# gkv856/speaker_embedding_GE2E_loss

Hardware: NVIDIA B200
Metric: GE2E fwd+bwd utterances/s (higher is better)
Workload: dtype tf32

## Files before the change

### speaker_embedding_ge2e_loss_b200/csrc/ge2e_tc.cu

```cuda
#include <cuda.h>
#include <cuda_fp16.h>
#include <cudaTypedefs.h>
#include <limits.h>
#include <stdlib.h>

#include <algorithm>
#include <cstring>
#include <type_traits>
#include <vector>

#include "ge2e_common.cuh"
#include "ge2e_tc_ptx.cuh"

namespace ge2e {

namespace {

using namespace ptx;

constexpr int kTile = 128;
constexpr int kUnit = 128;
constexpr int kSlabCols = 32;
constexpr int kSlabBytes = kTile * 128;
constexpr int kMaxSlabs = 8;
// ... 402 lines not shown
        if (DBG && (dbg & 8)) tr.mark();
        tc_fence_after();
      };
      auto next_bar = [&]() { return bar(BAR_FULL + (stage + 1 == kStages ? 0 : stage + 1)); };
      auto next_par = [&]() { return static_cast<uint32_t>(stage + 1 == kStages ? (phase ^ 1) : phase); };
      auto stage_done = [&](uint32_t probe) {
        __syncwarp();
        ready = __shfl_sync(0xffffffffu, probe, leader) != 0;
        advance();
      };
      auto mma1_stage = [&](uint32_t d_tmem, uint32_t idesc1, int rows_cta, int ks0, int nslab, bool first_of_seg) {
        if (kOpF16) {
          if (first_of_seg) {
            for (int sl = 0; sl < nslab; ++sl) {
              const int s = ks0 + sl, c = s % hs;
              mbar_wait(bar(BAR_A_FULL + c), sg & 1);
              if (kPlanes == 2 && s < hs) mbar_wait(bar(BAR_A_FULL + hs + c), sg & 1);
            }
          }
          stage_wait();
          uint32_t probe = 0;
          if (elect_leader(leader)) {
            probe = mbar_test(next_bar(), next_par());
            for (int sl = 0; sl < nslab; ++sl) {
              const int s = ks0 + sl, c = s % hs;
              const uint64_t db = dk | ((ring_smem + stage * kStageBytes + sl * rows_cta * 128) >> 4);
              umma_f16_ss4<CG>(d_tmem, dk | ((a_smem + c * kSlabBytes) >> 4), db, idesc1, s != 0);
              if (kPlanes == 2 && s < hs)
                umma_f16_ss4<CG>(d_tmem, dk | ((a_smem + (hs + c) * kSlabBytes) >> 4), db, idesc1, 1);
            }
            commit(BAR_EMPTY + stage);
          }
          stage_done(probe);
          return;
        }
        if (first_of_seg) {
          for (int sl = 0; sl < nslab; ++sl) mbar_wait(bar(BAR_A_FULL + ks0 + sl), sg & 1);
        }
        stage_wait();
        uint32_t probe = 0;
        if (elect_leader(leader)) {
          const uint64_t da = dk | ((a_smem + ks0 * kSlabBytes) >> 4);
          const uint64_t db = dk | ((ring_smem + stage * kStageBytes) >> 4);
          const uint32_t eb = bar(BAR_EMPTY + stage);
          if (nslab == 2)
            probe = umma_stage_ss<CG, 2>(d_tmem, da, db, kSlabBytes >> 4, static_cast<uint32_t>(rows_cta * 128) >> 4,
                                         idesc1, ks0 != 0, eb, next_bar(), next_par());
          else
            probe = umma_stage_ss<CG, 1>(d_tmem, da, db, 0, 0, idesc1, ks0 != 0, eb, next_bar(), next_par());
        }
        stage_done(probe);
      };
      const uint32_t idesc_unit = kOpF16 ? idesc_f16(kTile * CG, kUnit, 0, 0) : idesc_tf32(kTile * CG, kUnit, 0, 0);
      auto mma1_unit = [&](int iter, bool first_of_seg) {
        const uint32_t d_tmem = tmem + (iter & 1) * kUnit;
        for (int ks = 0; ks < oslabs; ks += 2)
          mma1_stage(d_tmem, idesc_unit, kUnit / CG, ks, min(2, oslabs - ks), first_of_seg);
        if (elect_one()) commit(BAR_S_FULL + (iter & 1));
        __syncwarp();
      };
      auto mma2_unit = [&](int iter, bool first) {
        const uint32_t a_tmem = tmem + (iter & 1) * kUnit;
        const uint32_t d_tmem = tmem + 2 * kUnit;
        for (int kc = 0; kc < kUnit / kM2; ++kc) {
          stage_wait();
          uint32_t probe = 0;
          if (PREC == PREC_F16) {
            if (elect_leader(leader)) {
              probe = mbar_test(next_bar(), next_par());
              const uint32_t a_hi = a_tmem + 64 * kc;
              const uint64_t db_hi = dmn | ((ring_smem + stage * kStageBytes) >> 4);
              umma_f16_ts2<CG>(d_tmem, a_hi, db_hi, idesc2, !(first && kc == 0));
              umma_f16_ts2<CG>(d_tmem, a_hi + 16, db_hi + 256, idesc2, 1);
              commit(BAR_EMPTY + stage);
            }
            stage_done(probe);
            continue;
          }
          if (kSplit) {
            if (elect_leader(leader)) {
              probe = mbar_test(next_bar(), next_par());
              const uint32_t a_hi = a_tmem + 64 * (kc >> 1) + 16 * (kc & 1), a_lo = a_hi + 32;
              const uint32_t sb = ring_smem + stage * kStageBytes;
              const uint64_t db_hi = dmn | (sb >> 4);
              const uint64_t db_lo = dmn | ((sb + (hs / CG) * kMma2Rows * 128) >> 4);
              umma_f16_ts2<CG>(d_tmem, a_hi, db_hi, idesc2, !(first && kc == 0));
              if (kPlanes == 2) {
                umma_f16_ts2<CG>(d_tmem, a_hi, db_lo, idesc2, 1);
                umma_f16_ts2<CG>(d_tmem, a_lo, db_hi, idesc2, 1);
              }
              commit(BAR_EMPTY + stage);
            }
            stage_done(probe);
            continue;
          }
          if (elect_leader(leader)) {
            const uint64_t db = dmn | ((ring_smem + stage * kStageBytes) >> 4);
            static_assert(kMma2Rows == 32, "umma_stage_ts issues 4 MMAs of 8 k-rows");
            probe = umma_stage_ts<CG>(d_tmem, a_tmem + kc * kMma2Rows, db, idesc2, !(first && kc == 0),
                                      bar(BAR_EMPTY + stage), next_bar(), next_par());
          }
          stage_done(probe);
        }
      };
      Walk wk = make_walk();
      int kind, og, s0, s1;
      for (; wk.next(p, kind, og, s0, s1); ++sg) {
        if (!kBwd) {
          for (int u = s0; u < s1; u += kStepUnits, ++it) {
            const int nu = min(kStepUnits, s1 - u);
            mbar_wait(bar(BAR_S_EMPTY + (it & 1)), ((it >> 1) & 1) ^ 1);
            tc_fence_after();
            const uint32_t d_tmem = tmem + (it & 1) * (kStepUnits * kUnit);
            const uint32_t idesc_step = kOpF16 ? idesc_f16(kTile * CG, nu * kUnit, 0, 0)
                                               : idesc_tf32(kTile * CG, nu * kUnit, 0, 0);
            for (int ks = 0; ks < oslabs; ++ks) mma1_stage(d_tmem, idesc_step, nu * kUnit / CG, ks, 1, u == s0);
            if (elect_one()) commit(BAR_S_FULL + (it & 1));
            __syncwarp();
            tr.mark();
          }
          if (elect_one()) commit(BAR_A_EMPTY);
          __syncwarp();
        } else {
          mma1_unit(it, true);
          for (int i = 0; i < s1 - s0; ++i, ++it) {
            if (i + 1 < s1 - s0) {
              mma1_unit(it + 1, false);
            } else {
              if (elect_one()) commit(BAR_A_EMPTY);
              __syncwarp();
            }
            tr.mark();
            if (i == 0 && sg > 0) { mbar_wait(bar(BAR_ACC_EMPTY), (sg - 1) & 1); tc_fence_after(); }
            mbar_wait(bar(BAR_G_FULL + (it & 1)), (it >> 1) & 1);
            tc_fence_after();
            tr.mark();
            mma2_unit(it, i == 0);
            tr.mark();
          }
          if (elect_one()) commit(BAR_ACC_FULL);
          __syncwarp();
        }
      }
    }
  } else if (warp >= kEpiWarp0) {
    const int ew = warp - kEpiWarp0;
    const int et = tid - kEpiWarp0 * 32;
    const int quarter = ew & 3, half = ew >> 2;
    const int trow = quarter * 32 + lane;
    const uint32_t lane_addr = static_cast<uint32_t>(quarter * 32) << 16;
    const float w = __ldg(p.w), b = __ldg(p.b), eps = p.eps;
    const float w2 = w * kLog2e, b2 = fmaf(w, eps, b) * kLog2e;
    const float bb = fmaf(w, eps, b);
    const float g = (kBwd && !RG && p.grad_out != nullptr) ? __ldg(p.grad_out) : 1.f;
    const float wg = w * g;
    float gamma = 1.f, inv_gamma = 1.f;
    auto gsign_of = [&](int buf, int w) -> uint32_t {
      if constexpr (RG) return tail->gsign[buf][w]; else return 0u;
    };
    const float m2 = b2 + fabsf(w2), c0 = -fabsf(w2);
    float dw_acc = 0.f, db_acc = 0.f, loss_acc = 0.f;
    int it = 0;
    const bool close_here = kBwd && !kSplit && (p.phases & PASS_ROWS);
    Tracer<DBG> tr((trow == 0 && half == 0) ? p.trace : nullptr, 2, kBwd ? 3 : 0);
    tr.mark();
    const uint32_t s_empty0 = lbar(BAR_S_EMPTY), g_full0 = lbar(BAR_G_FULL), acc_empty = lbar(BAR_ACC_EMPTY);
    auto arrive_leader = [&](uint32_t addr) {
      if (CG == 1) mbar_arrive(addr); else mbar_arrive_cluster(addr);
    };
    auto spin_until = [&](const int* ctr, int target) {
      unsigned long long t0 = 0;
      for (unsigned spins = 0;; ++spins) {
        int v;
        asm volatile("ld.acquire.gpu.global.s32 %0, [%1];" : "=r"(v) : "l"(ctr) : "memory");
        if (v >= target) break;
        if ((spins & 1023u) == 1023u) {
          const unsigned long long t = globaltimer_ns();
          if (t0 == 0) t0 = t;
          else if (t - t0 > 2000000000ull) __trap();
        }
      }
    };
    bool zero_seen = false;
    auto wait_zero_fill = [&]() {
      if (zero_seen) return;
      spin_until(p.ctr, static_cast<int>(gridDim.x));
      asm volatile("fence.proxy.async;" ::: "memory");
      zero_seen = true;
    };
    if (kBwd) {
      auto zfill = [&](float4* base, long long n4) {
        const long long z0 = n4 * blockIdx.x / gridDim.x, z1 = n4 * (blockIdx.x + 1) / gridDim.x;
        for (long long i = z0 + et; i < z1; i += kEpiThreads) base[i] = make_float4(0.f, 0.f, 0.f, 0.f);
      };
      if (p.zero_n4 > 0) zfill(p.zero_base, p.zero_n4);
      if (p.zero2_n4 > 0) zfill(p.zero2_base, p.zero2_n4);
      if (close_here) zfill(reinterpret_cast<float4*>(p.rowsum), (p.n_own[SEG_DE] + 3) / 4);
      if (et == 0) tail->rows_all_done = 0;
      __threadfence();
      named_bar_sync(1, kEpiThreads);
      if (et == 0) atomicAdd(p.ctr, 1);
    }

    int lift2 = kSplitLift;
    auto close_row = [&](int r) {
      const float cdv = __ldg(p.cos_diag + r);
      float stat, q;
      if (close_here) {
        const RowClose rc = close_softmax_row_log2(m2, __ldcg(p.rowsum + r), fmaf(cdv, w2, b2),
                                                   fmaf(w, cdv + eps, b), eps);
        stat = rc.stat; q = rc.q;
        p.row_stat_out[r] = stat;
        p.row_aux_out[r] = q;
        p.row_scale_out[r] = w / rc.z;
        if (p.per_row_out != nullptr) p.per_row_out[r] = rc.per;
        loss_acc += rc.per;
      } else {
        stat = __ldg(p.row_stat + r);
        q = __ldg(p.row_aux + r);
        if (kSplit && (p.phases & PASS_ROWS))
          p.row_scale_out[r] = w * exp2f(static_cast<float>(-(kSplitLift + split_extra_lift(q))));
      }
      if (p.phases & PASS_CENTROIDS) {
        if (RG) {
          const float gr = __ldg(p.grad_rows + r);
          dw_acc = fmaf(-q * gr, cdv + eps, dw_acc);
          db_acc -= gr * eps * expf(-stat);
        } else {
          dw_acc = fmaf(-q, cdv + eps, dw_acc);
          db_acc -= eps * expf(-stat);
        }
      }
    };
    auto close_rows = [&]() {
      const int U = p.n_own[SEG_DE];
      if (kSplit && (p.phases & PASS_CENTROIDS)) {
        if (RG) {
          float qm = 0.f, gm = 0.f;
          for (int r = et; r < U; r += kEpiThreads) {
            const float ga = fabsf(__ldg(p.grad_rows + r));
            qm = fmaxf(qm, __ldg(p.row_aux + r) * ga);
            gm = fmaxf(gm, ga);
          }
          qm = warp_max(qm);
          gm = warp_max(gm);
          if (lane == 0) { tail->red[ew] = qm; tail->red[kEpiWarps + ew] = gm; }
          named_bar_sync(1, kEpiThreads);
          qm = tail->red[0];
          gm = tail->red[kEpiWarps];
          for (int i = 1; i < kEpiWarps; ++i) { qm = fmaxf(qm, tail->red[i]); gm = fmaxf(gm, tail->red[kEpiWarps + i]); }
          gamma = gm;
          inv_gamma = gm > 0.f ? 1.f / gm : 0.f;
          lift2 = kSplitLift + split_extra_lift(qm * inv_gamma);
        } else {
          float qm = 0.f;
          for (int r = et; r < U; r += kEpiThreads) qm = fmaxf(qm, __ldg(p.row_aux + r));
          qm = warp_max(qm);
          if (lane == 0) tail->red[ew] = qm;
          named_bar_sync(1, kEpiThreads);
          qm = tail->red[0];
          for (int i = 1; i < kEpiWarps; ++i) qm = fmaxf(qm, tail->red[i]);
          lift2 = kSplitLift + split_extra_lift(qm);
        }
        named_bar_sync(1, kEpiThreads);
      }
      for (int r = blockIdx.x * kEpiThreads + et; r < U; r += gridDim.x * kEpiThreads) close_row(r);
      tr.mark();
    };
    static_assert(kUnit == kTile, "a pass-2 stream unit must be exactly one pass-1 owner tile");
    unsigned long long ready_wait_ns = 0;
    auto tile_ready = [&](int u) {
      if (*reinterpret_cast<volatile int*>(&tail->rows_all_done) != 0) return true;
      int v;
      asm volatile("ld.acquire.gpu.global.s32 %0, [%1];" : "=r"(v) : "l"(p.ctr + 2) : "memory");
      if (v >= p.OT[SEG_DE]) { tail->rows_all_done = 1; return true; }
      asm volatile("ld.acquire.gpu.global.s32 %0, [%1];" : "=r"(v) : "l"(p.seg_done + u) : "memory");
      return v >= p.ST[SEG_DE];
    };
    auto wait_tile = [&](int u) {
      if (tile_ready(u)) return;
      const unsigned long long t0 = DBG ? globaltimer_ns() : 0ull;
      spin_until(p.seg_done + u, p.ST[SEG_DE]);
      if (DBG) ready_wait_ns += globaltimer_ns() - t0;
    };
    bool closed = false;
    int sg_dc0 = -1;

    Walk wk = make_walk();
    int kind, og, s0, s1;
    for (int sg = 0; wk.next(p, kind, og, s0, s1); ++sg) {
      const bool is_dc = kBwd && kind == SEG_DC;
      if (kBwd && !close_here && is_dc && !closed) { close_rows(); closed = true; }
      if (DBG && is_dc && sg_dc0 < 0) { sg_dc0 = sg; tr.put(kTraceEvents - 2, globaltimer_ns()); }
      const int n_str = p.n_str[kind];
      const int ot = og * CG + cr;
      const bool tile_valid = ot < p.OT[kind];
      const int orow = ot * kTile + trow;
      const bool ovalid = orow < p.n_own[kind];
      int jg = -1;
      float cd = 0.f;
      int dlo = 0, dhi = 0;
      if (!is_dc) {
        if (ovalid) {
          jg = p.spk_offset + orow / p.M;
          if (!kBwd) cd = __ldg(p.cos_diag + orow);
        }
      } else {
        const int jl = orow - p.spk_offset;
        if (ovalid && jl >= 0 && (long long)jl * p.M < n_str) { dlo = jl * p.M; dhi = dlo + p.M; }
      }
      const float xd2 = fmaf(cd, w2, b2);
      float m2r = xd2, lsum = 0.f;
      float best = -INFINITY; int bestk = INT_MAX;
      float rs_acc = 0.f;
      float dw_seg = 0.f;
      auto lse2_of = [&](bool valid, float raw, float cdv) -> float {
        if (!valid) return INFINITY;
        if (!close_here) return raw * kLog2e;
        return close_softmax_row_log2(m2, raw, fmaf(cdv, w2, b2), fmaf(w, cdv + eps, b), eps).lse2;
      };
      auto lse2_raw = [&](int ur, float& raw, float& cdv) -> bool {
        if (ur >= n_str) return false;
        if (close_here) { raw = __ldcg(p.rowsum + ur); cdv = __ldg(p.cos_diag + ur); }
        else { raw = __ldg(p.row_stat + ur); cdv = 0.f; }
        return true;
      };
      float c0r = 0.f;
      if (kBwd && kSplit && !is_dc)
        c0r = ovalid ? (b2 + static_cast<float>(kSplitLift + split_extra_lift(__ldg(p.row_aux + orow)))) -
                           __ldg(p.row_stat + orow) * kLog2e
                     : -INFINITY;
      auto grad_of = [&](int ur) -> float { return (RG && ur < n_str) ? __ldg(p.grad_rows + ur) : 0.f; };
      auto stage_row = [&](int buf, bool valid, float raw, float cdv, float gr) {
        float l = lse2_of(valid, raw, cdv);
        if constexpr (RG) {
          l -= log2f(fabsf(gr) * inv_gamma);
          const uint32_t neg = __ballot_sync(0xffffffffu, gr < 0.f);
          if (lane == 0) tail->gsign[buf][quarter] = neg;
        }
        tail->lse_s[buf][trow] = l;
      };
      auto stage_lse = [&](int u, int buf) {
        if (close_here) wait_tile(u);
        float raw = 0.f, cdv = 0.f;
        const bool v = lse2_raw(u * kUnit + trow, raw, cdv);
        stage_row(buf, v, raw, cdv, grad_of(u * kUnit + trow));
      };
      if (is_dc && half == 0) stage_lse(wk.unit(0, s0, s1), it & 1);
      bool deferred = false;

      for (int i = 0; i < s1 - s0; i += kStepUnits, ++it) {
        const int u = wk.unit(i, s0, s1);
        const int nu = min(kStepUnits, s1 - s0 - i);
        const int buf = it & 1;
        float nraw = 0.f, ncd = 0.f, ngr = 0.f;
        bool nvalid = false;
        if (is_dc) {
          if (half == 0 && deferred) { stage_lse(u, buf); deferred = false; }
          named_bar_sync(1, kEpiThreads);
          if (half == 0 && i + 1 < s1 - s0) {
            const int un = wk.unit(i + 1, s0, s1);
            if (!close_here || tile_ready(un)) {
              nvalid = lse2_raw(un * kUnit + trow, nraw, ncd);
// ... 65 lines not shown
        for (int ch = half * nch; ch < (half + 1) * nch; ++ch) {
          const int cc = u * kUnit + ch * 32;
          uint32_t v[32];
          tmem_ld32(t_addr + ch * 32, v);
          tmem_ld_wait();
          if (!kBwd) {
            if (cc < n_str) {
              const bool tailc = cc + 32 > n_str;
              const bool diagc = static_cast<unsigned>(jg - cc) < 32u;
              if (VARIANT == GE2E_SOFTMAX) {
                float x[32];
#pragma unroll
                for (int i = 0; i < 32; ++i) x[i] = fmaf(__uint_as_float(v[i]), w2, b2);
                if (__any_sync(0xffffffffu, tailc || diagc)) {
#pragma unroll
                  for (int i = 0; i < 32; ++i)
                    if (cc + i == jg || cc + i >= n_str) x[i] = -INFINITY;
                }
                float cm = x[0];
#pragma unroll
                for (int i = 1; i < 32; ++i) cm = fmaxf(cm, x[i]);
                const float mn = fmaxf(m2r, cm);
                float sacc = 0.f;
#pragma unroll
                for (int i = 0; i < 32; ++i) sacc += ex2(x[i] - mn);
                lsum = fmaf(lsum, ex2(m2r - mn), sacc);
                m2r = mn;
              } else {
#pragma unroll
                for (int i = 0; i < 32; ++i) {
                  float sv = fmaf(__uint_as_float(v[i]), w, bb);
                  if (cc + i == jg || cc + i >= n_str) sv = -INFINITY;
                  if (sv > best) { best = sv; bestk = cc + i; }
                }
              }
            }
          } else {
            uint32_t gq[32];
            if (!is_dc) {
              const bool special = (cc + 32 > n_str) || (static_cast<unsigned>(jg - cc) < 32u);
              const bool any_special = __any_sync(0xffffffffu, special);
#pragma unroll
              for (int i = 0; i < 32; ++i) {
                float pr = ex2(fmaf(__uint_as_float(v[i]), w2, c0));
                if (any_special && (cc + i >= n_str || cc + i == jg)) pr = 0.f;
                rs_acc += pr;
                gq[i] = __float_as_uint(round_tf32(pr));
              }
            } else {
              const float4* ls4 = reinterpret_cast<const float4*>(&tail->lse_s[buf][ch * 32]);
              const uint32_t neg = gsign_of(buf, ch);
              const bool special = (cc < dhi) && (cc + 32 > dlo);
              const bool any_special = __any_sync(0xffffffffu, special);
#pragma unroll
              for (int i4 = 0; i4 < 8; ++i4) {
                const float4 l4 = ls4[i4];
                const float ls[4] = {l4.x, l4.y, l4.z, l4.w};
#pragma unroll
                for (int q = 0; q < 4; ++q) {
                  const int i = i4 * 4 + q;
                  const float dot = __uint_as_float(v[i]);
                  float pr = ex2(fmaf(dot, w2, b2) - ls[q]);
                  if (any_special && cc + i >= dlo && cc + i < dhi) pr = 0.f;
                  if (RG && ((neg >> i) & 1u)) pr = -pr;
                  dw_seg = fmaf(pr, dot + eps, dw_seg);
                  gq[i] = __float_as_uint(round_tf32(wg * pr));
                }
              }
            }
            tmem_st32(t_addr + ch * 32, gq);
          }
        }
        tr.mark();
        if (!kBwd) {
          tc_fence_before();
          __syncwarp();
          if (lane == 0) arrive_leader(s_empty0 + 8u * buf);
        } else {
          if (is_dc && half == 0 && i + 1 < s1 - s0 && !deferred) stage_row(buf ^ 1, nvalid, nraw, ncd, ngr);
          tmem_st_wait();
          tc_fence_before();
          __syncwarp();
          if (lane == 0) arrive_leader(g_full0 + 8u * buf);
        }
      }

      const bool full = (s0 == 0 && s1 == p.ST[kind]);
      if (!kBwd) {
        float2 mine;
        if (VARIANT == GE2E_SOFTMAX) mine = make_float2(m2r, lsum);
        else mine = make_float2(best, __int_as_float(bestk));
        if (half == 1) tail->xch[trow] = mine;
        named_bar_sync(1, kEpiThreads);
        const float2 theirs = tail->xch[trow];
        named_bar_sync(1, kEpiThreads);
        if (half == 0 && tile_valid) {
          auto fold = [&](float2 q) {
            if (VARIANT == GE2E_SOFTMAX) {
              const float mn = fmaxf(m2r, q.x);
              lsum = lsum * ex2(m2r - mn) + q.y * ex2(q.x - mn);
              m2r = mn;
            } else {
              const int qk = __float_as_int(q.y);
              if (q.x > best || (q.x == best && qk < bestk)) { best = q.x; bestk = qk; }
            }
          };
          fold(theirs);
          const int st = p.ST[SEG_DE];
          const int first_cl = cluster_of_pair(static_cast<long long>(og) * st, p.GP, NC);
          bool last = full;
          if (!full) {
            float2 part;
            if (VARIANT == GE2E_SOFTMAX) part = make_float2(m2r, lsum);
            else part = make_float2(best, __int_as_float(bestk));
            p.seg_part[(static_cast<size_t>(ot) * p.maxseg + (cl - first_cl)) * kTile + trow] = part;
            __threadfence();
            named_bar_sync(2, kTile);
            if (trow == 0) {
              const int done = atomicAdd(p.seg_done + ot, s1 - s0) + (s1 - s0);
              tail->flag = (done == st);
              if (done == st) p.seg_done[ot] = 0;
            }
            named_bar_sync(2, kTile);
            last = tail->flag != 0;
            if (last) {
              __threadfence();
              const int last_cl = cluster_of_pair(static_cast<long long>(og) * st + st - 1, p.GP, NC);
              const int nseg = last_cl - first_cl + 1;
              m2r = xd2; lsum = 0.f; best = -INFINITY; bestk = INT_MAX;
              for (int sgi = 0; sgi < nseg; ++sgi)
                fold(__ldcg(&p.seg_part[(static_cast<size_t>(ot) * p.maxseg + sgi) * kTile + trow]));
            }
          }
          if (last && ovalid) {
            const float Sd = fmaf(w, cd + eps, b);
            float per, stat, aux = 0.f;
            int ks = -1;
            if (VARIANT == GE2E_SOFTMAX) {
              const RowClose rc = close_softmax_row_log2(m2r, lsum, xd2, Sd, eps);
              stat = rc.stat; aux = rc.q; per = rc.per;
            } else {
              per = 1.f - 1.f / (1.f + expf(-Sd));
              stat = best;
              if (bestk != INT_MAX) { ks = bestk; per += 1.f / (1.f + expf(-best)); }
            }
            p.row_stat_out[orow] = stat;
            if (p.row_aux_out != nullptr) p.row_aux_out[orow] = aux;
            if (VARIANT == GE2E_CONTRAST && p.kstar_out != nullptr) p.kstar_out[orow] = ks;
            if (p.per_row_out != nullptr) p.per_row_out[orow] = per;
            loss_acc += per;
          }
        }
      } else {
        if (!is_dc && !close_here) {
        } else if (!is_dc) {
          if (et == 0) wait_zero_fill();
          named_bar_sync(1, kEpiThreads);
          if (ovalid) {
            const float old = atomicAdd(p.rowsum + orow, rs_acc);
            asm volatile("" ::"f"(old));
          }
          named_bar_sync(1, kEpiThreads);
          if (et == 0) {
            bool last = false;
            if (tile_valid) {
              __threadfence();
              last = atomicAdd(p.seg_done + ot, s1 - s0) + (s1 - s0) == p.ST[SEG_DE];
              if (last) { __threadfence(); atomicAdd(p.ctr + 2, 1); }
            }
            tail->flag = last;
          }
          named_bar_sync(1, kEpiThreads);
          if (tail->flag != 0) {
            __threadfence();
            if (et < kTile && ot * kTile + et < p.n_own[SEG_DE]) close_row(ot * kTile + et);
          }
          if (DBG && wk.kind == SEG_DE && wk.gp >= wk.end) tr.put(kTraceEvents - 3, globaltimer_ns());
        } else if (ovalid) {
          if (RG && kSplit) dw_acc += dw_seg * (exp2f(static_cast<float>(-lift2)) * gamma);
          else dw_acc += kSplit ? dw_seg * exp2f(static_cast<float>(-lift2)) : dw_seg;
        }
        mbar_wait(bar(BAR_ACC_FULL), sg & 1);
        tc_fence_after();
        tr.mark();
        fence_proxy_async_smem();
        const int ch0 = half ? kslabs / 2 : 0, ch1 = half ? kslabs : kslabs / 2;
        for (int ch = ch0; ch < ch1; ++ch) {
          uint32_t v[32];
          tmem_ld32(tmem + lane_addr + 2 * kUnit + ch * 32, v);
          tmem_ld_wait();
          if (kSplit && is_dc) {
            const float fs = (RG ? wg * gamma : wg) * exp2f(static_cast<float>(-lift2));
#pragma unroll
            for (int i = 0; i < 32; ++i) v[i] = __float_as_uint(__uint_as_float(v[i]) * fs);
          }
          const uint32_t row_smem = a_smem + ch * kSlabBytes + trow * 128;
#pragma unroll
          for (int c = 0; c < 8; ++c)
            asm volatile("st.shared.v4.b32 [%0], {%1, %2, %3, %4};" ::"r"(row_smem + ((c ^ (trow & 7)) << 4)),
                         "r"(v[4 * c]), "r"(v[4 * c + 1]), "r"(v[4 * c + 2]), "r"(v[4 * c + 3])
                         : "memory");
        }
        tc_fence_before();
        __syncwarp();
        if (lane == 0) arrive_leader(acc_empty);
        tr.mark();
        fence_proxy_async_smem();
        named_bar_sync(1, kEpiThreads);
        if (et == 0) {
          if (tile_valid) {
            const CUtensorMap* tm_out = &tms.out[kind];
            int row0 = ot * kTile;
            bool store = full;
            if (is_dc && p.peer_rows > 0) {
              const int r = row0 / p.peer_rows;
              tm_out = &tms.out_peer[r];
              row0 -= r * p.peer_rows;
              store = false;
            } else if (!full) {
              wait_zero_fill();
            }
            for (int ks = 0; ks < kslabs; ++ks) {
              if (store) tma_store_2d(tm_out, ks * kSlabCols, row0, a_smem + ks * kSlabBytes);
              else tma_reduce_add_2d(tm_out, ks * kSlabCols, row0, a_smem + ks * kSlabBytes);
              tma_store_commit();
            }
          }
          for (int ks = 0; ks < kslabs; ++ks) {
            if (tile_valid) tma_store_wait_read_pending(kslabs - 1 - ks);
            mbar_arrive(bar(BAR_A_FREE + ks));
          }
        }
      }
      tr.mark();
    }
    if (kBwd && !close_here && !closed) close_rows();
    if (DBG && kBwd) tr.put(kTraceEvents - 1, ready_wait_ns);

    if (!kBwd) {
      loss_acc = warp_sum(loss_acc);
      if (lane == 0) tail->red[ew] = loss_acc;
      named_bar_sync(1, kEpiThreads);
      if (ew == 0 && lane == 0) {
        float t = 0.f;
        for (int i = 0; i < kEpiWarps; ++i) t += tail->red[i];
        atomicAdd(p.loss_accum, t);
      }
    } else {
      loss_acc = warp_sum(loss_acc);
      dw_acc = warp_sum(dw_acc) * g;
      db_acc = warp_sum(db_acc) * g;
      if (lane == 0) { tail->red3[ew] = loss_acc; tail->red3[kEpiWarps + ew] = dw_acc; tail->red3[2 * kEpiWarps + ew] = db_acc; }
      named_bar_sync(1, kEpiThreads);
      if (et == 0) {
        float tl = 0.f, tw = 0.f, tb = 0.f;
        for (int i = 0; i < kEpiWarps; ++i) {
          tl += tail->red3[i]; tw += tail->red3[kEpiWarps + i]; tb += tail->red3[2 * kEpiWarps + i];
        }
        if (close_here) atomicAdd(p.loss_accum, tl);
        if (p.phases & PASS_CENTROIDS) { atomicAdd(p.dwdb + 0, tw); atomicAdd(p.dwdb + 1, tb); }
        if (p.stamps != nullptr) p.stamps[2 * blockIdx.x + 1] = globaltimer_ns();
        const bool last_out = atomicAdd(p.ctr + 1, 1) == static_cast<int>(gridDim.x) - 1;
        if (last_out) { atomicExch(p.ctr, 0); atomicExch(p.ctr + 1, 0); atomicExch(p.ctr + 2, 0); }
        tail->flag = last_out;
      }
      named_bar_sync(1, kEpiThreads);
      if (close_here && tail->flag != 0)
        for (int t = et; t < p.OT[SEG_DE]; t += kEpiThreads) p.seg_done[t] = 0;
    }
  }

  tc_fence_before();
  __syncthreads();
  if (CG > 1) cluster_sync_all();
  if (warp == 2) {
    if (CG == 1) tmem_dealloc<512>(tmem); else tmem_dealloc_2cta<512>(tmem);
  }
}

PFN_cuTensorMapEncodeTiled_v12000 get_encode() {
  static PFN_cuTensorMapEncodeTiled_v12000 fn = nullptr;
  if (fn == nullptr) {
    void* ptr = nullptr;
    cudaDriverEntryPointQueryResult qres;
    if (cudaGetDriverEntryPoint("cuTensorMapEncodeTiled", &ptr, cudaEnableDefault, &qres) == cudaSuccess &&
        qres == cudaDriverEntryPointSuccess)
      fn = reinterpret_cast<PFN_cuTensorMapEncodeTiled_v12000>(ptr);
  }
  return fn;
}

struct MapKey {
  const void* base; int rows, D, box, dims;
  bool operator==(const MapKey& o) const {
    return base == o.base && rows == o.rows && D == o.D && box == o.box && dims == o.dims;
  }
};
constexpr int kMapCache = 32;
struct MapCache { MapKey key[kMapCache]; CUtensorMap map[kMapCache]; int next = 0, used = 0; };
thread_local MapCache g_maps;

bool map_lookup(const MapKey& k, CUtensorMap* m) {
  for (int i = 0; i < g_maps.used; ++i)
    if (g_maps.key[i] == k) { *m = g_maps.map[i]; return true; }
  return false;
}
void map_store(const MapKey& k, const CUtensorMap& m) {
  g_maps.key[g_maps.next] = k;
  g_maps.map[g_maps.next] = m;
  g_maps.next = (g_maps.next + 1) % kMapCache;
  g_maps.used = std::min(g_maps.used + 1, kMapCache);
}

int make_map_2d(CUtensorMap* m, const float* base, int rows, int D, int box_rows) {
  const MapKey key{base, rows, D, box_rows, 2};
  if (map_lookup(key, m)) return GE2E_OK;
  auto enc = get_encode();
  if (enc == nullptr) return GE2E_ERR_LAUNCH;
  cuuint64_t dims[2] = {static_cast<cuuint64_t>(D), static_cast<cuuint64_t>(rows)};
  cuuint64_t strides[1] = {static_cast<cuuint64_t>(D) * 4};
  cuuint32_t box[2] = {kSlabCols, static_cast<cuuint32_t>(box_rows)};
  cuuint32_t estr[2] = {1, 1};
  CUresult r = enc(m, CU_TENSOR_MAP_DATA_TYPE_FLOAT32, 2, const_cast<float*>(base), dims, strides, box, estr,
                   CU_TENSOR_MAP_INTERLEAVE_NONE, CU_TENSOR_MAP_SWIZZLE_128B, CU_TENSOR_MAP_L2_PROMOTION_L2_256B,
                   CU_TENSOR_MAP_FLOAT_OOB_FILL_NONE);
  if (r == CUDA_SUCCESS) map_store(key, *m);
  return r == CUDA_SUCCESS ? GE2E_OK : GE2E_ERR_LAUNCH;
}

int make_map_3d(CUtensorMap* m, const float* base, int rows, int D, int box_slabs) {
  const MapKey key{base, rows, D, box_slabs, 3};
  if (map_lookup(key, m)) return GE2E_OK;
  auto enc = get_encode();
  if (enc == nullptr) return GE2E_ERR_LAUNCH;
  cuuint64_t dims[3] = {kSlabCols, static_cast<cuuint64_t>(rows), static_cast<cuuint64_t>(D / kSlabCols)};
  cuuint64_t strides[2] = {static_cast<cuuint64_t>(D) * 4, kSlabCols * 4};
  cuuint32_t box[3] = {kSlabCols, kMma2Rows, static_cast<cuuint32_t>(box_slabs)};
  cuuint32_t estr[3] = {1, 1, 1};
  CUresult r = enc(m, CU_TENSOR_MAP_DATA_TYPE_FLOAT32, 3, const_cast<float*>(base), dims, strides, box, estr,
                   CU_TENSOR_MAP_INTERLEAVE_NONE, CU_TENSOR_MAP_SWIZZLE_128B_ATOM_32B, CU_TENSOR_MAP_L2_PROMOTION_L2_256B,
                   CU_TENSOR_MAP_FLOAT_OOB_FILL_NONE);
  if (r == CUDA_SUCCESS) map_store(key, *m);
  return r == CUDA_SUCCESS ? GE2E_OK : GE2E_ERR_LAUNCH;
}

int make_map_h3(CUtensorMap* m, const void* base, int rows, int D, int box_rows) {
  const MapKey key{base, rows, D, box_rows, 15};
  if (map_lookup(key, m)) return GE2E_OK;
  auto enc = get_encode();
  if (enc == nullptr) return GE2E_ERR_LAUNCH;
  cuuint64_t dims[3] = {static_cast<cuuint64_t>(D), static_cast<cuuint64_t>(rows), 2};
  cuuint64_t strides[2] = {static_cast<cuuint64_t>(D) * 4, static_cast<cuuint64_t>(D) * 2};
  cuuint32_t box[3] = {64, static_cast<cuuint32_t>(box_rows), 1};
  cuuint32_t estr[3] = {1, 1, 1};
  CUresult r = enc(m, CU_TENSOR_MAP_DATA_TYPE_FLOAT16, 3, const_cast<void*>(base), dims, strides, box, estr,
                   CU_TENSOR_MAP_INTERLEAVE_NONE, CU_TENSOR_MAP_SWIZZLE_128B, CU_TENSOR_MAP_L2_PROMOTION_L2_256B,
                   CU_TENSOR_MAP_FLOAT_OOB_FILL_NONE);
  if (r == CUDA_SUCCESS) map_store(key, *m);
  return r == CUDA_SUCCESS ? GE2E_OK : GE2E_ERR_LAUNCH;
}
int make_map_h4(CUtensorMap* m, const void* base, int rows, int D, int box_chunks, int planes) {
  const int box_rows = planes == 1 ? 64 : kMma2Rows;
  const MapKey key{base, rows, D, box_chunks, 12 + planes};
  if (map_lookup(key, m)) return GE2E_OK;
  auto enc = get_encode();
  if (enc == nullptr) return GE2E_ERR_LAUNCH;
  cuuint64_t dims[4] = {64, static_cast<cuuint64_t>(rows), static_cast<cuuint64_t>(D / 64), 2};
  cuuint64_t strides[3] = {static_cast<cuuint64_t>(D) * 4, 128, static_cast<cuuint64_t>(D) * 2};
  cuuint32_t box[4] = {64, static_cast<cuuint32_t>(box_rows), static_cast<cuuint32_t>(box_chunks),
                       static_cast<cuuint32_t>(planes)};
  cuuint32_t estr[4] = {1, 1, 1, 1};
  CUresult r = enc(m, CU_TENSOR_MAP_DATA_TYPE_FLOAT16, 4, const_cast<void*>(base), dims, strides, box, estr,
                   CU_TENSOR_MAP_INTERLEAVE_NONE, CU_TENSOR_MAP_SWIZZLE_128B, CU_TENSOR_MAP_L2_PROMOTION_L2_256B,
                   CU_TENSOR_MAP_FLOAT_OOB_FILL_NONE);
  if (r == CUDA_SUCCESS) map_store(key, *m);
  return r == CUDA_SUCCESS ? GE2E_OK : GE2E_ERR_LAUNCH;
}

int make_map_h2(CUtensorMap* m, const void* base, int rows, int D, int box_rows) {
  const MapKey key{base, rows, D, box_rows, 16};
  if (map_lookup(key, m)) return GE2E_OK;
  auto enc = get_encode();
  if (enc == nullptr) return GE2E_ERR_LAUNCH;
  cuuint64_t dims[2] = {static_cast<cuuint64_t>(D), static_cast<cuuint64_t>(rows)};
  cuuint64_t strides[1] = {static_cast<cuuint64_t>(D) * 2};
  cuuint32_t box[2] = {64, static_cast<cuuint32_t>(box_rows)};
  cuuint32_t estr[2] = {1, 1};
  CUresult r = enc(m, CU_TENSOR_MAP_DATA_TYPE_FLOAT16, 2, const_cast<void*>(base), dims, strides, box, estr,
                   CU_TENSOR_MAP_INTERLEAVE_NONE, CU_TENSOR_MAP_SWIZZLE_128B, CU_TENSOR_MAP_L2_PROMOTION_L2_256B,
                   CU_TENSOR_MAP_FLOAT_OOB_FILL_NONE);
  if (r == CUDA_SUCCESS) map_store(key, *m);
  return r == CUDA_SUCCESS ? GE2E_OK : GE2E_ERR_LAUNCH;
}

__global__ void __launch_bounds__(256)
to_f16_kernel(const float4* __restrict__ a, uint2* __restrict__ a16, long long na4, const float4* __restrict__ b,
              uint2* __restrict__ b16, long long nb4) {
  pdl_wait();
  pdl_trigger();
  const long long stride = static_cast<long long>(gridDim.x) * blockDim.x;
  for (long long i = static_cast<long long>(blockIdx.x) * blockDim.x + threadIdx.x; i < na4 + nb4; i += stride) {
    const float4 v = (i < na4) ? __ldcg(a + i) : __ldcg(b + (i - na4));
    const __half2 h0 = __floats2half2_rn(v.x, v.y), h1 = __floats2half2_rn(v.z, v.w);
    uint2 o;
    o.x = *reinterpret_cast<const uint32_t*>(&h0); o.y = *reinterpret_cast<const uint32_t*>(&h1);
    if (i < na4) a16[i] = o; else b16[i - na4] = o;
  }
}

int g_hybrid_mode = 0;

unsigned long long* g_trace = nullptr;
int g_trace_mode = -1;
int g_trace_fine = 0;
unsigned long long* g_stamps = nullptr;

constexpr int kMaxDevices = 64;
int current_device() {
  int dev = 0;
  cudaGetDevice(&dev);
  return dev;
}

int sm_count() {
  static int n[kMaxDevices] = {0};
  const int dev = current_device();
  if (dev < 0 || dev >= kMaxDevices) return 148;
  if (n[dev] == 0) {
    cudaDeviceGetAttribute(&n[dev], cudaDevAttrMultiProcessorCount, dev);
    if (n[dev] <= 0) n[dev] = 148;
  }
  return n[dev];
}

int pick_cg(int D) { return ((D / kSlabCols) % 2 != 0) ? 1 : 2; }

template <int MODE, int VARIANT, int CG>
int max_clusters() {
  constexpr bool DBG = false;
  static int cache[kMaxDevices] = {0};
  const int dev = current_device();
  const bool cacheable = dev >= 0 && dev < kMaxDevices;
  if (cacheable && cache[dev] != 0) return cache[dev];
  int n = 0;
  {
    cudaLaunchConfig_t cfg{};
    cfg.gridDim = dim3(sm_count() / CG * CG);
    cfg.blockDim = dim3(kThreadsTc);
    cfg.dynamicSmemBytes = kSmemBytes;
    cudaLaunchAttribute at[1];
    at[0].id = cudaLaunchAttributeClusterDimension;
    at[0].val.clusterDim.x = CG; at[0].val.clusterDim.y = 1; at[0].val.clusterDim.z = 1;
    cfg.attrs = at; cfg.numAttrs = 1;
    cudaFuncSetAttribute(tc_strip_kernel<MODE, VARIANT, CG, PREC_TF32, DBG>, cudaFuncAttributeMaxDynamicSharedMemorySize,
                         (int)kSmemBytes);
    if (cudaOccupancyMaxActiveClusters(&n, tc_strip_kernel<MODE, VARIANT, CG, PREC_TF32, DBG>, &cfg) != cudaSuccess) n = 0;
    (void)cudaGetLastError();
  }
  if (n <= 0) return 0;
  n = std::min(n, kMaxClusters);
  if (cacheable) cache[dev] = n;
  return n;
}

struct Layout {
  int OT, ST, CG, OG, NC, maxseg;
  long long GP;
  size_t done_bytes, part_bytes;
  bool whole;
};

Layout make_layout(int n_own, int n_str, int cg, int max_cl) {
  Layout L{};
  L.OT = (n_own + kTile - 1) / kTile;
  L.ST = (n_str + kUnit - 1) / kUnit;
  L.CG = cg;
  L.OG = (L.OT + L.CG - 1) / L.CG;
  L.GP = static_cast<long long>(L.OG) * L.ST;
  L.NC = static_cast<int>(std::min<long long>(std::max(max_cl, 1), L.GP));
  const long long per = L.GP / L.NC;
  L.maxseg = static_cast<int>(std::min<long long>(L.ST, L.ST / per + 2));
  L.done_bytes = (static_cast<size_t>(L.OT) * sizeof(int) + 255) & ~static_cast<size_t>(255);
  L.part_bytes = static_cast<size_t>(L.OT) * L.maxseg * kTile * sizeof(float2);
  L.whole = (L.GP % L.NC == 0) && (per % L.ST == 0);
  return L;
}

constexpr int kStraddle = 3;
bool cut_pass(long long GP, int OG, int ST, int NC, const double* delay, int* out) {
  if (GP == 0) { for (int c = 0; c <= NC; ++c) out[c] = 0; return false; }
  const long long level = (GP + NC - 1) / NC;
  const long long cost_whole = static_cast<long long>((OG + NC - 1) / NC) * ST;
  const long long cost_flat = level + ((GP % NC == 0 && level % ST == 0) ? 0 : kStraddle);
  long long cost_assigned = LLONG_MAX;
  if (OG <= NC) {
    const int n_min = NC / OG;
    cost_assigned = (ST + n_min - 1) / n_min;
  }
  auto split = [&](int c0, int c1, long long base, long long units) {
    const int n = c1 - c0;
    double dsum = 0;
    for (int c = c0; c < c1; ++c) dsum += delay ? delay[c] : 0.0;
    const double K = (static_cast<double>(units) + dsum) / n;
    double wsum = 0, cum = 0;
    for (int c = c0; c < c1; ++c) wsum += std::max(0.25, K - (delay ? delay[c] : 0.0));
    for (int c = c0; c < c1; ++c) {
      out[c] = static_cast<int>(base + static_cast<long long>(units * (cum / wsum) + 0.5));
      cum += std::max(0.25, K - (delay ? delay[c] : 0.0));
    }
  };
  if (cost_assigned <= cost_whole && cost_assigned <= cost_flat && OG < NC) {
    for (int g = 0; g < OG; ++g) {
      const int c0 = static_cast<int>(static_cast<long long>(g) * NC / OG);
      const int c1 = static_cast<int>(static_cast<long long>(g + 1) * NC / OG);
      split(c0, c1, static_cast<long long>(g) * ST, ST);
    }
    out[NC] = static_cast<int>(GP);
    return NC > OG;
  }
  if (cost_whole <= cost_flat) {
    for (int c = 0; c <= NC; ++c) out[c] = static_cast<int>((static_cast<long long>(c) * OG / NC) * ST);
    return false;
  }
  split(0, NC, 0, GP);
  out[NC] = static_cast<int>(GP);
  return true;
}

constexpr double kPassSwitch = 2.5;

struct StepModel {
  int NC = 0;
  double start2[kMaxClusters];
  std::vector<double> ready;
};

void model_pass1(const int* de, int NC, int STe, int cg, int STc, StepModel* m) {
  m->NC = NC;
  m->ready.assign(STc, 0.0);
  for (int c = 0; c < NC; ++c) {
    double t = 0;
    for (long long gp = de[c]; gp < de[c + 1];) {
      const long long og = gp / STe, end = std::min<long long>(de[c + 1], (og + 1) * STe);
      t += static_cast<double>(end - gp) + (gp > de[c] ? kStraddle : 0);
      for (int k = 0; k < cg; ++k) {
        const long long tile = og * cg + k;
        if (tile < STc) m->ready[tile] = std::max(m->ready[tile], t);
      }
      gp = end;
    }
    m->start2[c] = de[c + 1] > de[c] ? t + kPassSwitch : 0.0;
  }
}

double model_finish(const StepModel& m, int c, long long a, long long b, int STc, int rot) {
  double t = m.start2[c];
  const long long n = b - a;
  for (long long i = 0; i < n; ++i) {
    long long gp = a + i + rot;
    if (gp >= b) gp -= n;
    if (i > 0 && gp / STc != (gp - 1) / STc && rot == 0) t += kStraddle;
    t = std::max(t, m.ready[gp % STc]) + 1.0;
  }
  return t;
}

int best_rotation(const StepModel& m, long long a, long long b, int STc) {
  if (b - a < 2 || a / STc != (b - 1) / STc) return 0;
  long long late = a;
  for (long long gp = a; gp < b; ++gp)
    if (m.ready[gp % STc] >= m.ready[late % STc]) late = gp;
  return static_cast<int>((late + 1 - a) % (b - a));
}

bool greedy_pass2(const StepModel& m, long long GP, int STc, double T, int* out) {
  const int NC = m.NC;
  const long long level = (GP + NC - 1) / NC;
  long long gp = 0;
  for (int c = 0; c < NC; ++c) {
    out[c] = static_cast<int>(gp);
    double late = -1, t_in = m.start2[c];
    long long n = 0, nlate = 0;
    bool crossed = false;
    while (gp < GP) {
      const bool cross = n > 0 && gp % STc == 0;
      if (cross && STc >= level && crossed) break;
      const double r = m.ready[gp % STc];
      const double t1 = std::max(t_in + (cross ? kStraddle : 0), r) + 1.0;
      const double l = std::max(late, r);
      const long long nl = (r > late) ? 1 : nlate + (r == late ? 1 : 0);
      const double est = (crossed || cross) ? t1 : std::max(m.start2[c] + static_cast<double>(n + 1), l + nl);
      if (est > T) break;
      crossed = crossed || cross; t_in = t1; late = l; nlate = nl; ++n; ++gp;
    }
  }
  out[NC] = static_cast<int>(GP);
  return gp == GP;
}

double model_makespan(const StepModel& m, const int* dc, int STc, const unsigned char* rot, double* finish) {
  double worst = 0;
  for (int c = 0; c < m.NC; ++c) {
    const double f = std::max(m.start2[c], model_finish(m, c, dc[c], dc[c + 1], STc, rot[c]));
    if (finish != nullptr) finish[c] = f;
    worst = std::max(worst, f);
  }
  return worst;
}

bool cut_pass2_barrier(const int* de, int NC, long long GPe, long long GPc, int OGc, int STc, int* dc) {
  double delay[kMaxClusters];
  long long busiest = 0;
  for (int c = 0; c < NC; ++c) busiest = std::max<long long>(busiest, de[c + 1] - de[c]);
  for (int c = 0; c < NC; ++c) {
    const long long load = de[c + 1] - de[c];
    delay[c] = (GPe > 0 && load > 0) ? std::max<double>(0.0, kStraddle - static_cast<double>(busiest - load)) : 0.0;
  }
  return cut_pass(GPc, OGc, STc, NC, GPe > 0 ? delay : nullptr, dc);
}

struct SchedKey {
  int OGe, STe, OGc, STc, phases, max_cl, cg, rows_closed;
  bool operator==(const SchedKey& o) const {
    return OGe == o.OGe && STe == o.STe && OGc == o.OGc && STc == o.STc && phases == o.phases &&
           max_cl == o.max_cl && cg == o.cg && rows_closed == o.rows_closed;
  }
};
struct SchedEntry { SchedKey key; StepSched S; int NC; bool dep, dcp; };
thread_local SchedEntry g_sched[4];
thread_local int g_sched_used = 0, g_sched_next = 0;

int make_step_sched(int OGe, int STe, int OGc, int STc, int phases, int max_cl, int cg, bool rows_closed,
                    StepSched* S, bool* de_partial, bool* dc_partial, double* model_out = nullptr,
                    double* barrier_makespan = nullptr) {
  const SchedKey key{OGe, STe, OGc, STc, phases, max_cl, cg, rows_closed ? 1 : 0};
  if (model_out == nullptr && barrier_makespan == nullptr)
    for (int i = 0; i < g_sched_used; ++i)
      if (g_sched[i].key == key) {
        *S = g_sched[i].S; *de_partial = g_sched[i].dep; *dc_partial = g_sched[i].dcp;
        return g_sched[i].NC;
      }
  const long long GPe = (phases & PASS_ROWS) ? static_cast<long long>(OGe) * STe : 0;
  const long long GPc = (phases & PASS_CENTROIDS) ? static_cast<long long>(OGc) * STc : 0;
  const int NC = static_cast<int>(std::max<long long>(1, std::min<long long>(max_cl, std::max(GPe, GPc))));
  std::memset(S->dc_rot, 0, sizeof(S->dc_rot));
  *de_partial = cut_pass(GPe, OGe, STe, NC, nullptr, S->de);
  const bool both = phases == (PASS_ROWS | PASS_CENTROIDS);
  *dc_partial = cut_pass2_barrier(S->de, NC, both ? GPe : 0, GPc, OGc, STc, S->dc);
  if (both && rows_closed) {
    StepModel m;
    model_pass1(S->de, NC, STe, cg, STc, &m);
    if (barrier_makespan != nullptr) {
      StepModel mb = m;
      double p1 = 0;
      for (int c = 0; c < NC; ++c) p1 = std::max(p1, mb.start2[c] - kPassSwitch);
      for (int c = 0; c < NC; ++c) mb.start2[c] = std::max(p1, mb.start2[c]);
      std::fill(mb.ready.begin(), mb.ready.end(), 0.0);
      *barrier_makespan = model_makespan(mb, S->dc, STc, S->dc_rot, nullptr);
    }
    double best = model_makespan(m, S->dc, STc, S->dc_rot, nullptr);
    int cand[kMaxClusters + 1];
    unsigned char rot[kMaxClusters];
    double lo = 0, hi = best;
    for (int c = 0; c < NC; ++c) lo = std::max(lo, std::min(m.start2[c], hi));
    lo = std::max(lo, static_cast<double>(GPc) / NC);
    const bool small = GPc <= 64LL * NC;
    for (int iter = 0; small && iter < 24 && hi - lo > 0.02; ++iter) {
      const double mid = 0.5 * (lo + hi);
      if (greedy_pass2(m, GPc, STc, mid, cand)) hi = mid; else lo = mid;
    }
    if (small && greedy_pass2(m, GPc, STc, hi, cand)) {
      for (int c = 0; c < NC; ++c) rot[c] = static_cast<unsigned char>(std::min(255, best_rotation(m, cand[c], cand[c + 1], STc)));
      for (int c = 0; c < NC; ++c)
        if (cand[c + 1] - cand[c] > 255) rot[c] = 0;
      const double got = model_makespan(m, cand, STc, rot, nullptr);
      if (got < best) {
        best = got;
        std::memcpy(S->dc, cand, sizeof(int) * (NC + 1));
        std::memcpy(S->dc_rot, rot, sizeof(rot[0]) * NC);
        *dc_partial = false;
        for (int c = 0; c <= NC; ++c) *dc_partial |= (S->dc[c] % STc) != 0;
      }
// ... 304 lines not shown
```

Before: 176.3 million.

## Interleave epilogue TMEM drain with per-slab TMA stores and offload row publish

The epilogue now drains accumulator slabs in pairs, with the two halves interleaved. After each pair, the TMA store or reduce for those slabs is issued right away instead of waiting until the whole tile has been drained, so stores overlap the remaining TMEM loads. The row-sum publish, completion counting and row close are moved after the accumulator release and run only on the second half of the epilogue warps, using a separate named barrier. The first half handles slab-free signalling in parallel. Some scalars are now reloaded late to cut register pressure, and the pass-switch heuristic threshold is lowered, which changes which schedule the planner picks. The cost is more barrier rounds per tile.

```diff
diff --git a/speaker_embedding_ge2e_loss_b200/csrc/ge2e_tc.cu b/speaker_embedding_ge2e_loss_b200/csrc/ge2e_tc.cu
--- a/speaker_embedding_ge2e_loss_b200/csrc/ge2e_tc.cu
+++ b/speaker_embedding_ge2e_loss_b200/csrc/ge2e_tc.cu
@@ -578,8 +578,8 @@
     const float w = __ldg(p.w), b = __ldg(p.b), eps = p.eps;
     const float w2 = w * kLog2e, b2 = fmaf(w, eps, b) * kLog2e;
     const float bb = fmaf(w, eps, b);
-    const float g = (kBwd && !RG && p.grad_out != nullptr) ? __ldg(p.grad_out) : 1.f;
-    const float wg = w * g;
+    auto grad_scalar = [&]() { return (kBwd && !RG && p.grad_out != nullptr) ? __ldg(p.grad_out) : 1.f; };
+    const float wg = w * grad_scalar();
     float gamma = 1.f, inv_gamma = 1.f;
     auto gsign_of = [&](int buf, int w) -> uint32_t {
       if constexpr (RG) return tail->gsign[buf][w]; else return 0u;
@@ -589,6 +589,7 @@
     int it = 0;
     const bool close_here = kBwd && !kSplit && (p.phases & PASS_ROWS);
     Tracer<DBG> tr((trow == 0 && half == 0) ? p.trace : nullptr, 2, kBwd ? 3 : 0);
+    Tracer<DBG> tr_pub((trow == 0 && half == 1) ? p.trace : nullptr, 2, 3);
     tr.mark();
     const uint32_t s_empty0 = lbar(BAR_S_EMPTY), g_full0 = lbar(BAR_G_FULL), acc_empty = lbar(BAR_ACC_EMPTY);
     auto arrive_leader = [&](uint32_t addr) {
@@ -634,7 +635,7 @@
       float stat, q;
       if (close_here) {
         const RowClose rc = close_softmax_row_log2(m2, __ldcg(p.rowsum + r), fmaf(cdv, w2, b2),
-                                                   fmaf(w, cdv + eps, b), eps);
+                                                   fmaf(w, cdv + eps, __ldg(p.b)), eps);
         stat = rc.stat; q = rc.q;
         p.row_stat_out[r] = stat;
         p.row_aux_out[r] = q;
@@ -1006,16 +1007,64 @@
           }
         }
       } else {
-        if (!is_dc && !close_here) {
-        } else if (!is_dc) {
+        const bool publish = close_here && !is_dc;
+        if (publish) {
           if (et == 0) wait_zero_fill();
           named_bar_sync(1, kEpiThreads);
-          if (ovalid) {
-            const float old = atomicAdd(p.rowsum + orow, rs_acc);
-            asm volatile("" ::"f"(old));
-          }
+          if (ovalid) atomicAdd(p.rowsum + orow, rs_acc);
+        } else if (is_dc && ovalid) {
+          if (RG && kSplit) dw_acc += dw_seg * (exp2f(static_cast<float>(-lift2)) * gamma);
+          else dw_acc += kSplit ? dw_seg * exp2f(static_cast<float>(-lift2)) : dw_seg;
+        }
+        mbar_wait(bar(BAR_ACC_FULL), sg & 1);
+        tc_fence_after();
+        tr.mark();
+        auto flush_slab = [&](int ks) {
+          const CUtensorMap* tm_out = &tms.out[kind];
+          int row0 = ot * kTile;
+          bool store = full;
+          if (is_dc && p.peer_rows > 0) {
+            const int r = row0 / p.peer_rows;
+            tm_out = &tms.out_peer[r];
+            row0 -= r * p.peer_rows;
+            store = false;
+          } else if (!full) {
+            wait_zero_fill();
+          }
+          if (store) tma_store_2d(tm_out, ks * kSlabCols, row0, a_smem + ks * kSlabBytes);
+          else tma_reduce_add_2d(tm_out, ks * kSlabCols, row0, a_smem + ks * kSlabBytes);
+          tma_store_commit();
+        };
+        fence_proxy_async_smem();
+        for (int j = 0; 2 * j < kslabs; ++j) {
+          const int ch = 2 * j + half;
+          if (ch < kslabs) {
+            uint32_t v[32];
+            tmem_ld32(tmem + lane_addr + 2 * kUnit + ch * 32, v);
+            tmem_ld_wait();
+            if (kSplit && is_dc) {
+              const float fs = (RG ? wg * gamma : wg) * exp2f(static_cast<float>(-lift2));
+#pragma unroll
+              for (int i = 0; i < 32; ++i) v[i] = __float_as_uint(__uint_as_float(v[i]) * fs);
+            }
+            const uint32_t row_smem = a_smem + ch * kSlabBytes + trow * 128;
+#pragma unroll
+            for (int c = 0; c < 8; ++c)
+              asm volatile("st.shared.v4.b32 [%0], {%1, %2, %3, %4};" ::"r"(row_smem + ((c ^ (trow & 7)) << 4)),
+                           "r"(v[4 * c]), "r"(v[4 * c + 1]), "r"(v[4 * c + 2]), "r"(v[4 * c + 3])
+                           : "memory");
+          }
+          fence_proxy_async_smem();
           named_bar_sync(1, kEpiThreads);
-          if (et == 0) {
+          if (et == 0 && tile_valid)
+            for (int ks = 2 * j; ks < min(2 * j + 2, kslabs); ++ks) flush_slab(ks);
+        }
+        tc_fence_before();
+        __syncwarp();
+        if (lane == 0) arrive_leader(acc_empty);
+        tr.mark();
+        if (publish && half == 1) {
+          if (et == kTile) {
             bool last = false;
             if (tile_valid) {
               __threadfence();
@@ -1023,63 +1072,14 @@
               if (last) { __threadfence(); atomicAdd(p.ctr + 2, 1); }
             }
             tail->flag = last;
-          }
-          named_bar_sync(1, kEpiThreads);
+            if (DBG && wk.kind == SEG_DE && wk.gp >= wk.end) tr_pub.put(kTraceEvents - 3, globaltimer_ns());
+          }
+          named_bar_sync(3, kTile);
           if (tail->flag != 0) {
             __threadfence();
-            if (et < kTile && ot * kTile + et < p.n_own[SEG_DE]) close_row(ot * kTile + et);
-          }
-          if (DBG && wk.kind == SEG_DE && wk.gp >= wk.end) tr.put(kTraceEvents - 3, globaltimer_ns());
-        } else if (ovalid) {
-          if (RG && kSplit) dw_acc += dw_seg * (exp2f(static_cast<float>(-lift2)) * gamma);
-          else dw_acc += kSplit ? dw_seg * exp2f(static_cast<float>(-lift2)) : dw_seg;
-        }
-        mbar_wait(bar(BAR_ACC_FULL), sg & 1);
-        tc_fence_after();
-        tr.mark();
-        fence_proxy_async_smem();
-        const int ch0 = half ? kslabs / 2 : 0, ch1 = half ? kslabs : kslabs / 2;
-        for (int ch = ch0; ch < ch1; ++ch) {
-          uint32_t v[32];
-          tmem_ld32(tmem + lane_addr + 2 * kUnit + ch * 32, v);
-          tmem_ld_wait();
-          if (kSplit && is_dc) {
-            const float fs = (RG ? wg * gamma : wg) * exp2f(static_cast<float>(-lift2));
-#pragma unroll
-            for (int i = 0; i < 32; ++i) v[i] = __float_as_uint(__uint_as_float(v[i]) * fs);
-          }
-          const uint32_t row_smem = a_smem + ch * kSlabBytes + trow * 128;
-#pragma unroll
-          for (int c = 0; c < 8; ++c)
-            asm volatile("st.shared.v4.b32 [%0], {%1, %2, %3, %4};" ::"r"(row_smem + ((c ^ (trow & 7)) << 4)),
-                         "r"(v[4 * c]), "r"(v[4 * c + 1]), "r"(v[4 * c + 2]), "r"(v[4 * c + 3])
-                         : "memory");
-        }
-        tc_fence_before();
-        __syncwarp();
-        if (lane == 0) arrive_leader(acc_empty);
-        tr.mark();
-        fence_proxy_async_smem();
-        named_bar_sync(1, kEpiThreads);
-        if (et == 0) {
-          if (tile_valid) {
-            const CUtensorMap* tm_out = &tms.out[kind];
-            int row0 = ot * kTile;
-            bool store = full;
-            if (is_dc && p.peer_rows > 0) {
-              const int r = row0 / p.peer_rows;
-              tm_out = &tms.out_peer[r];
-              row0 -= r * p.peer_rows;
-              store = false;
-            } else if (!full) {
-              wait_zero_fill();
-            }
-            for (int ks = 0; ks < kslabs; ++ks) {
-              if (store) tma_store_2d(tm_out, ks * kSlabCols, row0, a_smem + ks * kSlabBytes);
-              else tma_reduce_add_2d(tm_out, ks * kSlabCols, row0, a_smem + ks * kSlabBytes);
-              tma_store_commit();
-            }
-          }
+            if (ovalid) close_row(orow);
+          }
+        } else if (et == 0) {
           for (int ks = 0; ks < kslabs; ++ks) {
             if (tile_valid) tma_store_wait_read_pending(kslabs - 1 - ks);
             mbar_arrive(bar(BAR_A_FREE + ks));
@@ -1102,6 +1102,7 @@
       }
     } else {
       loss_acc = warp_sum(loss_acc);
+      const float g = grad_scalar();
       dw_acc = warp_sum(dw_acc) * g;
       db_acc = warp_sum(db_acc) * g;
       if (lane == 0) { tail->red3[ew] = loss_acc; tail->red3[kEpiWarps + ew] = dw_acc; tail->red3[2 * kEpiWarps + ew] = db_acc; }
@@ -1381,7 +1382,7 @@
   return true;
 }
 
-constexpr double kPassSwitch = 2.5;
+constexpr double kPassSwitch = 1.8;
 
 struct StepModel {
   int NC = 0;
```

After: 175.1 million (median of 6 runs). No clear change (-0.6%).
